# abdel-habib/mmg-clip

Hardware: AMD Instinct MI355X
Metric: image-text pairs/sec (global batch) (higher is better)
Workload: dtype bf16; 1 GPU; C2: train_binary_class_clf, ConvNeXt-tiny 1024x1024x1 + BERT-base S=77, LinearProjection 768->512, CLIPLoss, AdamW, all parameters trained; global_batch=256, per_gpu_batch=256, micro_batch=256, streams=text tower on a side stream, parallelism=dp1, loss_scope=local, text_dropout=HF training-mode dropout live (hidden 0.1, atte…

## Files before the change

### include/mmgclip_hip.h

```cpp
#ifndef MMGCLIP_HIP_H
#define MMGCLIP_HIP_H

#ifdef __cplusplus
extern "C" {
#endif

typedef void* mmg_stream_t;

int mmg_abi_version(void);
const char* mmg_last_error(void);
const char* mmg_target_arch(void);
int mmg_device_cu_count(void);
int mmg_set_kernel_notes(int on);
const char* mmg_last_kernel(void);
const char* mmg_gemm_plan(int op, int M, int N, int K, int cus);


int mmg_l2norm_fwd(const float* x, float* y, float* norm, int rows, int D, mmg_stream_t stream);
int mmg_l2norm_bwd(const float* y, const float* norm, const float* dy, float* dx, int rows, int D,
                   mmg_stream_t stream);

int mmg_clip_rows_fwd(const float* X, const float* Y, const float* scale, int n_loc, int N, int D, int diag_off,
                      float* lse, float* pos, float* logits, int ldl, mmg_stream_t stream);

// ... 38 lines not shown

int mmg_gelu_fwd_bf16(const void* x, void* y, long long n, mmg_stream_t stream);
int mmg_act_grad_bf16(const void* dy, const void* pre, void* out, long long n, int kind, mmg_stream_t stream);
int mmg_cast_f32_bf16(const float* x, void* y, long long n, mmg_stream_t stream);
int mmg_cast_bf16_f32(const void* x, float* y, long long n, mmg_stream_t stream);
int mmg_transpose_cast_bf16(const float* src, int R, int C, const float* rowscale, void* dst, int ldd,
                            mmg_stream_t stream);

int mmg_avgpool_fwd(const void* x, float* y, int n, int HW, int C, mmg_stream_t stream);
int mmg_avgpool_bwd(const float* dy, void* dx, int n, int HW, int C, mmg_stream_t stream);

int mmg_view_pool_fwd(const float* feat, const int* offsets, float* out, int* argmax, int S, int C, int mode, mmg_stream_t stream);
int mmg_view_pool_bwd(const float* dout, const int* offsets, const int* argmax, float* dfeat, int S, int V, int C, int mode,
                      mmg_stream_t stream);

int mmg_patchify(const float* img, void* out, int n, int Cin, int H, int W, int P, int Kp, int scale16,
                 mmg_stream_t stream);
int mmg_patchify_aug(const void* img, int src_kind, void* out, int n, int Cin, int H, int W, int P, int Kp, int scale16,
                     const int* geom, const float* tone, mmg_stream_t stream);

int mmg_adamw_step(float* p, const float* g, float* m, float* v, void* p_bf16, long long n, float lr, float beta1,
                   float beta2, float eps, float weight_decay, int step, float grad_scale, mmg_stream_t stream);


int mmg_grad_sumsq_partials(long long n);
int mmg_grad_sumsq(const float* g, long long n, double* partials, int n_partials, mmg_stream_t stream);
int mmg_grad_clip_finalize(const double* partials, int n, float max_norm, float* out, int* skipped, mmg_stream_t stream);
int mmg_adamw_step_guarded(float* p, const float* g, float* m, float* v, void* p_bf16, long long n, float lr, float beta1,
                           float beta2, float eps, float weight_decay, int step, const float* clip, const int* skipped,
                           mmg_stream_t stream);
int mmg_adamw_step_groups(float* p, const float* g, float* m, float* v, long long n, const unsigned char* chunk_group, int n_groups,
                          const float* group_lr, const float* group_wd, float beta1, float beta2, float eps, int step,
                          const float* clip, const int* skipped, mmg_stream_t stream);

int mmg_layerscale_finalize(const float* W2, const float* b2, const float* gamma, const float* dW2raw,
                            const float* db2raw, float* dW2, float* db2, float* dgamma, int C, int K,
                            mmg_stream_t stream);
int mmg_grad_relayout(const float* src, float* dst, int mode, int R, int CI, int KH, int KW, int ld_src,
                      mmg_stream_t stream);

int mmg_image_swap(void* x, const int* pairs, const int* pairs_host, int k, int n, long long rows, int C, mmg_stream_t stream);
int mmg_image_copy(const void* src, void* dst, int first, int count, int n, long long rows, int C, mmg_stream_t stream);
int mmg_scaled_add_f32(float* dst, const float* src, float alpha, long long n, mmg_stream_t stream);

int mmg_dropout_fwd(const float* x, float* y, void* keep, long long n, float p, long long seed, mmg_stream_t stream);
int mmg_dropout_bwd(const float* dy, const void* keep, float* dx, long long n, float p, mmg_stream_t stream);


int mmg_dwconv7_nhwc(const void* x, const float* w, const float* bias, const void* add, void* y, int n, int H, int W,
                     int C, int flip, mmg_stream_t stream);
int mmg_dwconv7_nhwc_mfma(const void* x, const float* w, const float* bias, const void* add, void* y, int n, int H, int W,
                          int C, int flip, mmg_stream_t stream);
int mmg_dwconv7_wgrad(const void* x, const void* dy, float* dw, float* dbias, int n, int H, int W, int C,
                      mmg_stream_t stream);


long long mmg_cnblock_packed_elems(int C, int backward);
int mmg_cnblock_pack_weights(const float* w1, const float* w2, const float* gamma, void* packed, int C, int backward,
                             mmg_stream_t stream);
int mmg_cnblock_mlp_fwd(const void* xd, const float* ln_w, const float* ln_b, float eps, const void* packed,
                        const float* b1, const float* b2, const float* gamma, const void* residual, void* y, void* hpre,
                        void* xln, void* gact, float* mean, float* rstd, int hpre_kind, long long M, int C, mmg_stream_t stream);

int mmg_cnblock_mlp_bwd_supported(int C);
int mmg_cnblock_mlp_bwd(const void* dy, const void* xd, const float* ln_w, const float* ln_b, float eps,
                        const void* packed_bwd, const float* b1, const void* hpre, void* dh, void* g, void* xln,
                        void* dxln, float* mean, float* rstd, float* ln_dw, float* ln_db, long long M, int C,
                        mmg_stream_t stream);

int mmg_cnblock_bwdw_supported(int C);
long long mmg_cnblock_bwdw_packed_elems(int C);
int mmg_cnblock_bwdw_pack(const float* w1, const float* w2, const float* ln_w, const float* ln_b, const float* layer_scale,
                          const float* b1, void* packed, float* b1f, int C, mmg_stream_t stream);
int mmg_cnblock_bwdw(const void* dy, const void* xd, const float* ln_w, const float* ln_b, float eps, const void* packed,
                     const float* b1f, void* dd, float* dW1, float* db1, float* dW2raw, float* db2raw, float* ln_dw,
                     float* ln_db, long long M, int C, mmg_stream_t stream);

int mmg_stem_supported(int C, int kp);
int mmg_stem_fwd(const void* p0, const void* w, const float* bias, const float* ln_w, const float* ln_b, float eps, void* x,
                 float* mean, float* rstd, long long M, int C, int kp, mmg_stream_t stream);
int mmg_stem_bwd(const void* dx, const void* p0, const void* w, const float* bias, const float* ln_w, const float* mean,
                 const float* rstd, float* dW, float* db, float* ln_dw, float* ln_db, long long M, int C, int kp,
                 mmg_stream_t stream);


int mmg_greedy_threshold_labels(const float* sim, int ld, int n, float threshold, long long* labels, int* counts, int* k_out,
                                mmg_stream_t stream);

int mmg_cluster_mean_cols_fwd(const float* logits, int ld, int n, int N, const long long* labels, const int* counts, int k,
                              float* out, int ldo, mmg_stream_t stream);
int mmg_cluster_mean_cols_bwd(const float* dout, int ldo, int n, int N, const long long* labels, const int* counts,
                              float* dlogits, int ld, mmg_stream_t stream);

int mmg_clip_labelled_rows_fwd(const float* X, const float* Y, const float* scale, const long long* row_label, int n_loc, int M,
                               int D, float* lse, float* pos, mmg_stream_t stream);
int mmg_clip_labelled_rows_bwd_row(const float* X, const float* Y, const float* scale, const float* lse_row,
                                   const long long* row_label, const float* gout, float coef, int n_loc, int M, int D,
                                   int accumulate, float* dX, float* dscale, mmg_stream_t stream);
int mmg_clip_labelled_rows_bwd_col(const float* X, const float* Y, const float* scale, const float* lse_col,
                                   const long long* col_label, const long long* row_key, int key_off, const int* counts,
                                   int n_counts, const float* gout, float coef, int n_loc, int M, int D, int accumulate,
                                   float* dX, mmg_stream_t stream);
int mmg_cluster_centroids(const float* T, const long long* labels, int N, int D, int k, float* out, mmg_stream_t stream);


int mmg_gemm_nt_fp8(const void* A, int lda, const void* B, int ldb, void* C, int ldc, int M, int N, int K,
                    const float* bias, const float* colscale, const void* residual, int ldr, void* aux_out, int ldao,
                    int epi, int out_kind, float alpha, const float* alpha_dev, mmg_stream_t stream);


int mmg_quantize_e5m2_bf16(const void* src, long long n, float* amax, void* dst, float* scales, mmg_stream_t stream);
int mmg_quantize_e5m2_bf16_delayed(const void* src, long long n, const float* amax_prev, float* amax_next, void* dst, float* scales,
                                   mmg_stream_t stream);
int mmg_quantize_e5m2_colsum_bf16(const void* src, int M, int C, const float* amax_prev, float* amax_next, void* dst, float* scales,
                                  float* colsum, mmg_stream_t stream);
int mmg_gemm_nt_fp8_bwd(const void* A, int lda, int a_e5m2, const void* B, int ldb, void* C, int ldc, int M, int N, int K,
                        const void* aux_in, int ldai, int epi, int out_kind, float alpha, const float* alpha_dev,
                        const float* alpha_dev2, mmg_stream_t stream);
int mmg_gemm_tn_fp8(const void* A, int lda, int a_e5m2, const void* B, int ldb, float* C, int ldc, int M, int N1, int N2,
                    float alpha, const float* alpha_dev, float* colsum_a, mmg_stream_t stream);

int mmg_absmax_f32(const float* src, long long n, float* amax, mmg_stream_t stream);
int mmg_quantize_e4m3_f32(const float* src, long long n, const float* amax, void* dst, float* scales, mmg_stream_t stream);

int mmg_layernorm_fwd_fp8(const void* x, int ldx, const float* gamma, const float* beta, float eps, void* y8, int ldy,
                          float* mean, float* rstd, int M, int C, mmg_stream_t stream);


int mmg_im2col_nhwc(const void* x, void* col, int n, int H, int W, int C, int KH, int KW, int stride, int pad, int Kp,
                    mmg_stream_t stream);
int mmg_col2im_nhwc(const void* dcol, void* dx, int n, int H, int W, int C, int KH, int KW, int stride, int pad, int Kp,
                    mmg_stream_t stream);
int mmg_maxpool3x3s2_nhwc(const void* x, void* y, int n, int H, int W, int C, mmg_stream_t stream);
int mmg_bn_stats_f64(const void* x, int M, int C, double* sum, double* sumsq, mmg_stream_t stream);
int mmg_bn_finalize_f64(const double* sum, const double* sumsq, int M, int C, const float* gamma, const float* beta, float eps,
                        float momentum, float* running_mean, float* running_var, int train, float* mean, float* rstd,
                        float* scale, float* shift, mmg_stream_t stream);
int mmg_bn_apply(const void* x, const float* scale, const float* shift, const void* residual, void* y, int M, int C, int relu,
                 mmg_stream_t stream);
int mmg_bn_bwd_reduce(const void* dy, const void* x, const void* out, const float* mean, const float* rstd, int M, int C,
                      float* sum_g, float* sum_gx, mmg_stream_t stream);
int mmg_bn_bwd_apply(const void* dy, const void* x, const void* out, const float* mean, const float* rstd, const float* gamma,
                     const float* sum_g, const float* sum_gx, int M, int C, void* dx, void* dres, float* dgamma, float* dbeta,
                     mmg_stream_t stream);


int mmg_attention_fwd(const void* qkv, int ld, const long long* mask, void* ctx, int ldc, float* lse, int B, int S,
                      int heads, int Hd, float scale, mmg_stream_t stream);
int mmg_attention_bwd(const void* qkv, int ld, const long long* mask, const void* ctx, int ldc, const float* lse,
                      const void* dctx, int lddc, void* dqkv, int lddq, int B, int S, int heads, int Hd, float scale,
                      mmg_stream_t stream);

int mmg_attention_long_fwd(const void* qkv, int ld, const long long* mask, void* ctx, int ldc, float* lse, int B, int S,
                           int heads, int Hd, float scale, mmg_stream_t stream);
int mmg_attention_long_bwd(const void* qkv, int ld, const long long* mask, const void* ctx, int ldc, const float* lse,
                           const void* dctx, int lddc, void* dqkv, int lddq, float* delta_ws, int B, int S, int heads,
                           int Hd, float scale, mmg_stream_t stream);

int mmg_attention_varlen_fwd(const void* qkv, int ld, const int* cu_seqlens, void* ctx, int ldc, float* lse, int B, int S_max,
                             int heads, int Hd, float scale, mmg_stream_t stream);
int mmg_attention_varlen_bwd(const void* qkv, int ld, const int* cu_seqlens, const void* ctx, int ldc, const float* lse,
                             const void* dctx, int lddc, void* dqkv, int lddq, int B, int S_max, int heads, int Hd,
                             float scale, mmg_stream_t stream);

int mmg_attention_dropout_fwd(const void* qkv, int ld, const long long* mask, const int* cu_seqlens, void* ctx, int ldc,
                              float* lse, int B, int S, int heads, int Hd, float scale, float p, unsigned long long seed,
// ... 35 lines not shown
```

### mmg-clip_amd/mmgclip/kernels.py

```python
import ctypes
import os

import torch

from . import _hip
from ._hip import call, ptr, stream
from .profile import PROFILE

BF16 = torch.bfloat16


def layernorm_fwd(x, gamma, beta, eps, patch_hw=None, want_stats=True):
    M, C = x.shape
    if patch_hw is None:
        y = torch.empty(M, C, device=x.device, dtype=BF16)
        patch, H, W = 0, 0, 0
    else:
        H, W = patch_hw
        y = torch.empty((M // (H * W)) * (H // 2) * (W // 2), 4 * C, device=x.device, dtype=BF16)
        patch = 1
    mean = torch.empty(M, device=x.device, dtype=torch.float32) if want_stats else None
    rstd = torch.empty(M, device=x.device, dtype=torch.float32) if want_stats else None
    PROFILE.timed("layernorm_fwd_kernel", 8.0 * M * C, 4 * M * C,
                  lambda: call("mmg_layernorm_fwd", ptr(x), x.stride(0), ptr(gamma), ptr(beta), float(eps), ptr(y), y.stride(0), ptr(mean),
# ... 152 lines not shown


def view_pool_fwd(feat, offsets, S, mode, out=None, argmax=None):
    V, C = feat.shape
    assert feat.dtype == torch.float32 and feat.is_contiguous() and offsets.dtype == torch.int32 and offsets.numel() == S + 1
    _hip.require_gpu(feat, offsets)
    y = out if out is not None else torch.empty(S, C, device=feat.device, dtype=torch.float32)
    if mode == 1 and argmax is None:
        argmax = torch.empty(S, C, device=feat.device, dtype=torch.int32)
    call("mmg_view_pool_fwd", ptr(feat), ptr(offsets), ptr(y), ptr(argmax) if mode == 1 else None, S, C, mode, stream())
    return y, (argmax if mode == 1 else None)


def view_pool_bwd(dout, offsets, argmax, V, mode, out=None):
    S, C = dout.shape
    assert dout.dtype == torch.float32 and dout.is_contiguous() and offsets.dtype == torch.int32 and offsets.numel() == S + 1
    _hip.require_gpu(dout, offsets)
    dx = out if out is not None else torch.empty(V, C, device=dout.device, dtype=torch.float32)
    call("mmg_view_pool_bwd", ptr(dout), ptr(offsets), ptr(argmax), ptr(dx), S, V, C, mode, stream())
    return dx


PIXEL_KINDS = {torch.float32: 0, torch.uint16: 1, torch.uint8: 2}


def stack_images(images):
    if images[0].dtype == torch.uint16:
        return torch.stack([t.view(torch.int16) for t in images]).view(torch.uint16)
    return torch.stack(list(images))


def patchify(img, P, Kp, scale16, geom=None, tone=None):
    n, Cin, H, W = img.shape
    if img.dtype not in PIXEL_KINDS:
        raise TypeError(f"pixels must be float32 in [0, 1], uint16 or uint8, got {img.dtype}")
    assert img.is_contiguous(), "pixels must be contiguous [n, Cin, H, W]"
    _hip.require_gpu(img, geom, tone)
    out = torch.empty(n * (H // P) * (W // P), Kp, device=img.device, dtype=BF16)
    if img.dtype == torch.float32 and geom is None and tone is None:
        call("mmg_patchify", ptr(img), ptr(out), n, Cin, H, W, P, Kp, 1 if scale16 else 0, stream())
        return out
    assert geom is None or (geom.dtype == torch.int32 and geom.is_contiguous() and tuple(geom.shape) == (n, 4)), "geom: int32 [n, 4]"
    assert tone is None or (tone.dtype == torch.float32 and tone.is_contiguous() and tuple(tone.shape) == (n, 2)), "tone: fp32 [n, 2]"
    call("mmg_patchify_aug", ptr(img), PIXEL_KINDS[img.dtype], ptr(out), n, Cin, H, W, P, Kp, 1 if scale16 else 0, ptr(geom), ptr(tone),
         stream())
    return out


def stem_supported(C, kp):
    return bool(_hip.load().mmg_stem_supported(int(C), int(kp)))


def stem_fused_enabled():
    return os.environ.get("MMG_STEM_FUSED", "1") != "0"


def stem_fwd(p0, w, bias, ln_w, ln_b, eps, want_stats=True):
    M, kp = p0.shape
    C = w.shape[0]
    assert p0.dtype == BF16 and w.dtype == BF16 and p0.is_contiguous() and w.is_contiguous() and w.shape[1] == kp
    _hip.require_gpu(p0, w, bias, ln_w, ln_b)
    x = torch.empty(M, C, device=p0.device, dtype=BF16)
    mean = torch.empty(M, device=p0.device, dtype=torch.float32) if want_stats else None
    rstd = torch.empty(M, device=p0.device, dtype=torch.float32) if want_stats else None
    PROFILE.timed("stem_fwd_kernel", 2.0 * M * C * kp, 2 * M * (kp + C) + (8 * M if want_stats else 0) + 2 * C * kp,
                  lambda: call("mmg_stem_fwd", ptr(p0), ptr(w), ptr(bias), ptr(ln_w), ptr(ln_b), float(eps), ptr(x), ptr(mean), ptr(rstd),
                               M, C, kp, stream()), f"M={M} C={C} kp={kp}" + (" +stats" if want_stats else ""))
    return x, mean, rstd


def stem_bwd(dx, p0, w, bias, ln_w, mean, rstd, dW, db, ln_dw, ln_db):
    M, kp = p0.shape
    C = w.shape[0]
    assert dx.dtype == BF16 and p0.dtype == BF16 and dx.is_contiguous() and p0.is_contiguous() and tuple(dx.shape) == (M, C)
    assert mean.dtype == rstd.dtype == torch.float32 and mean.numel() == rstd.numel() == M
    for t, n in ((dW, C * kp), (db, C), (ln_dw, C), (ln_db, C)):
        assert t.dtype == torch.float32 and t.is_contiguous() and t.numel() == n
    _hip.require_gpu(dx, p0, w, bias, ln_w, mean, rstd, dW, db, ln_dw, ln_db)
    PROFILE.timed("stem_bwd_kernel", 2.0 * M * C * kp, 2 * M * (kp + C) + 8 * M + 6 * C * kp,
                  lambda: call("mmg_stem_bwd", ptr(dx), ptr(p0), ptr(w), ptr(bias), ptr(ln_w), ptr(mean), ptr(rstd), ptr(dW), ptr(db),
                               ptr(ln_dw), ptr(ln_db), M, C, kp, stream()), f"M={M} C={C} kp={kp}")


def adamw_step(p, g, m, v, p16, lr, beta1, beta2, eps, wd, step, grad_scale=1.0):
    call("mmg_adamw_step", ptr(p), ptr(g), ptr(m), ptr(v), ptr(p16), p.numel(), float(lr), float(beta1), float(beta2),
         float(eps), float(wd), int(step), float(grad_scale), stream())


def grad_sumsq_partials(n):
    return int(_hip.load().mmg_grad_sumsq_partials(int(n)))


def grad_sumsq(g, partials, offset=0, count=None):
    assert g.dtype == torch.float32 and g.is_contiguous() and partials.dtype == torch.float64 and partials.is_contiguous()
    _hip.require_gpu(g, partials)
    count = grad_sumsq_partials(g.numel()) if count is None else int(count)
    assert 0 <= offset and offset + count <= partials.numel()
    call("mmg_grad_sumsq", ptr(g), g.numel(), ptr(partials[offset:]) if count else ptr(partials), count, stream())


def grad_clip_finalize(partials, n, max_norm, out, skipped=None):
    assert partials.dtype == torch.float64 and out.dtype == torch.float32 and out.numel() >= 3 and n <= partials.numel()
    assert skipped is None or (skipped.dtype == torch.int32 and skipped.numel() >= 1)
    _hip.require_gpu(partials, out, skipped)
    call("mmg_grad_clip_finalize", ptr(partials), int(n), 0.0 if max_norm is None else float(max_norm), ptr(out), ptr(skipped), stream())


def adamw_step_guarded(p, g, m, v, p16, lr, beta1, beta2, eps, wd, step, clip, skipped=None):
    assert clip.dtype == torch.float32 and clip.numel() >= 3 and (skipped is None or skipped.dtype == torch.int32)
    call("mmg_adamw_step_guarded", ptr(p), ptr(g), ptr(m), ptr(v), ptr(p16), p.numel(), float(lr), float(beta1), float(beta2),
         float(eps), float(wd), int(step), ptr(clip), ptr(skipped), stream())


ADAMW_MAX_GROUPS = 128


def adamw_step_groups(p, g, m, v, chunk_group, group_lr, group_wd, beta1, beta2, eps, step, clip=None, skipped=None):
    n_groups = len(group_lr)
    assert len(group_wd) == n_groups and chunk_group.dtype == torch.uint8 and chunk_group.is_contiguous()
    assert chunk_group.numel() * 64 == p.numel() == g.numel() == m.numel() == v.numel()
    assert clip is None or (clip.dtype == torch.float32 and clip.numel() >= 3)
    assert skipped is None or skipped.dtype == torch.int32
    _hip.require_gpu(p, g, m, v, chunk_group, clip, skipped)
    lrs = (ctypes.c_float * max(n_groups, 1))(*[float(x) for x in group_lr])
    wds = (ctypes.c_float * max(n_groups, 1))(*[float(x) for x in group_wd])
    call("mmg_adamw_step_groups", ptr(p), ptr(g), ptr(m), ptr(v), p.numel(), ptr(chunk_group), n_groups, lrs, wds, float(beta1),
         float(beta2), float(eps), int(step), ptr(clip), ptr(skipped), stream())


def dwconv_mfma_pays(n, H, W, C, flip):
    return H * W >= 96 * 96 and C <= 256


def dwconv7(x, w49, bias, n, H, W, C, add=None, flip=False, out=None):
    y = out if out is not None else torch.empty(n * H * W, C, device=x.device, dtype=BF16)
    px = n * H * W * C
    mode = os.environ.get("MMG_DWCONV_MFMA", "auto")
    if mode == "1" or (mode == "auto" and dwconv_mfma_pays(n, H, W, C, flip)):
        PROFILE.timed("dwconv7_mfma_kernel", 98.0 * px, (6 if add is not None else 4) * px,
                      lambda: call("mmg_dwconv7_nhwc_mfma", ptr(x), ptr(w49), ptr(bias), ptr(add), ptr(y), n, H, W, C, 1 if flip else 0, stream()),
                      f"n={n} {H}x{W} C={C}" + (" +add" if add is not None else ""))
        return y
    fam = "dwconv7_rows2_kernel" if os.environ.get("MMG_DWCONV_ROWS2", "1") != "0" else "dwconv7_kernel"
    PROFILE.timed(fam, 98.0 * px, (6 if add is not None else 4) * px,
                  lambda: call("mmg_dwconv7_nhwc", ptr(x), ptr(w49), ptr(bias), ptr(add), ptr(y), n, H, W, C, 1 if flip else 0, stream()),
                  f"n={n} {H}x{W} C={C}" + (" +add" if add is not None else ""))
    return y


def dwconv7_wgrad(x, dy, dw49, dbias, n, H, W, C):
    px = n * H * W * C
    fam = "dwconv7_wgrad_rows2_kernel" if os.environ.get("MMG_DWCONV_ROWS2", "1") != "0" else "dwconv7_wgrad_kernel"
    PROFILE.timed(fam, 98.0 * px, 4 * px,
                  lambda: call("mmg_dwconv7_wgrad", ptr(x), ptr(dy), ptr(dw49), ptr(dbias), n, H, W, C, stream()), f"n={n} {H}x{W} C={C}")


def cnblock_supported(C):
    return C in (96, 128, 192, 256, 384, 512)


def cnblock_pack(w1, w2, gamma=None, backward=False):
    C = w1.shape[1]
    backward = int(backward)
    n = _hip.load().mmg_cnblock_packed_elems(C, backward)
    if n <= 0:
        raise ValueError(f"fused CNBlock MLP: C={C} is not supported")
# ... 225 lines not shown
```

### mmg-clip_amd/mmgclip/networks/convnext.py

```python
import ctypes
import os

import torch
import torch.nn as nn

from .. import _hip
from .. import kernels as K
from .. import linalg as L
from .._hip import call, ptr, stream
from ..params import backward_finished, last_backward
from . import convnext_sd as SD
from .convnext_plan import BlockSaved, Knobs, decide_saves, fused_forward, plan_block, saving_form
from .tower import Tower, as_pixels, augment_tables, backward_parts, conv_weight_rows, fold_conv_grad, forward_parts

CONFIGS = {
    "tiny": dict(depths=(3, 3, 9, 3), dims=(96, 192, 384, 768)),
    "small": dict(depths=(3, 3, 27, 3), dims=(96, 192, 384, 768)),
    "base": dict(depths=(3, 3, 27, 3), dims=(128, 256, 512, 1024)),
}
LN_EPS = 1e-6


def _fused_save_maxc():
    return int(os.environ.get("MMG_MLP_FUSED_SAVE_MAXC", "384"))


class LayerNorm2d(nn.LayerNorm):
    """Parameter container with torchvision's name; the arithmetic runs in mmg_layernorm_fwd."""


class CNBlock(nn.Module):
    def __init__(self, dim, layer_scale=1e-6):
        super().__init__()
        self.block = nn.Sequential(
            nn.Conv2d(dim, dim, kernel_size=7, padding=3, groups=dim, bias=True),
            nn.Identity(),
            nn.LayerNorm(dim, eps=LN_EPS),
            nn.Linear(dim, 4 * dim, bias=True),
            nn.GELU(),
            nn.Linear(4 * dim, dim, bias=True),
            nn.Identity(),
        )
        self.layer_scale = nn.Parameter(torch.ones(dim, 1, 1) * layer_scale)


def build_features(variant="tiny", in_chans=1):
    cfg = CONFIGS[variant]
    dims, depths = cfg["dims"], cfg["depths"]
    layers = [nn.Sequential(nn.Conv2d(in_chans, dims[0], kernel_size=4, stride=4, bias=True), LayerNorm2d(dims[0], eps=LN_EPS))]
    for i, (d, n) in enumerate(zip(dims, depths)):
        layers.append(nn.Sequential(*[CNBlock(d) for _ in range(n)]))
        if i < 3:
            layers.append(nn.Sequential(LayerNorm2d(d, eps=LN_EPS), nn.Conv2d(d, dims[i + 1], kernel_size=2, stride=2)))
    feats = nn.Sequential(*layers)
    for m in feats.modules():
        if isinstance(m, (nn.Conv2d, nn.Linear)):
            nn.init.trunc_normal_(m.weight, std=0.02)
            if m.bias is not None:
                nn.init.zeros_(m.bias)
    return feats


class _TorchvisionLayout(nn.Module):

    def __init__(self, variant, in_chans):
        super().__init__()
        self.features = build_features(variant, in_chans)
        self.avgpool = nn.AdaptiveAvgPool2d(1)


class ConvNextTower(Tower):

    def __init__(self, variant="tiny", in_chans=1, scale16=True, micro_batch=64, fused_mlp=None, checkpoint=False, fp8=False,
                 fp8_min_channels=None, stochastic_depth_prob=0.0, augment=None):
        super().__init__()
        self.set_augment(augment)
        self.stochastic_depth_prob = SD.check_rate(stochastic_depth_prob)
        self.next_drop_seed = None
        self._drop_seeds = SD.DropSeeds()
        self.variant, self.in_chans, self.scale16, self.micro_batch = variant, in_chans, scale16, micro_batch
        self.fused_mlp = (os.environ.get("MMG_FUSED_MLP", "1") != "0") if fused_mlp is None else bool(fused_mlp)
        self.fused_bwd_saved_h = os.environ.get("MMG_FUSED_MLP_BWD_SAVED_H", "0") == "1"
        self.bwdw = os.environ.get("MMG_BWDW", "1") != "0"
        self.save_ln_mode = os.environ.get("MMG_SAVE_LN", "auto")
        self.save_ln = self.save_ln_mode == "1"
        self.save_gelu_mode = os.environ.get("MMG_SAVE_GELU", "auto")
        self.save_gelu = self.save_gelu_mode == "1"
        self.save_dgelu = os.environ.get("MMG_SAVE_DGELU", "1") != "0"
        self.checkpoint = checkpoint
        self.fp8 = bool(fp8)
        self.fp8_bwd_mode = os.environ.get("MMG_FP8_BWD", "auto")
        self.fp8_bwd = self.fp8_bwd_mode != "0"
        self.fp8_bwd_now = False
        self.fp8_delayed = os.environ.get("MMG_FP8_DELAYED", "1") != "0"
        self._e5m2_state = {}
        self.fp8_min_channels = int(os.environ.get("MMG_FP8_MIN_C", "256" if self.fp8_bwd else "512")) if fp8_min_channels is None else int(fp8_min_channels)
        self.dims, self.depths = CONFIGS[variant]["dims"], CONFIGS[variant]["depths"]
        self.model = _TorchvisionLayout(variant, in_chans)
        self.model_output_dimension = self.dims[-1]
        self.kp = (16 * in_chans + 31) // 32 * 32
        self.plan = None

    def _bound(self):
        self._pname = {id(m): "features." + n for n, m in self.model.features.named_modules()}

    def _g(self, mod, leaf):
        return self._arena.g(self._pname[id(mod)] + "." + leaf)
# ... 114 lines not shown
            s0 = L.gemm_nt(p0, wc["stem.w"], bias=f[0][0].bias.data)
            x, mean, rstd = K.layernorm_fwd(s0, f[0][1].weight.data, f[0][1].bias.data, LN_EPS, want_stats=save)
        if save:
            saved["stem"] = (p0, s0, mean, rstd)
        for si, p in enumerate(plan):
            mlp = self._fwd_fused if fused_forward(p, save) else self._fwd_gemm
            for bi, blk in enumerate(f[1 + 2 * si]):
                key = f"{si}.{bi}"
                step = steps[b] if steps is not None else None
                b += 1
                if step is None or step.n_k == n:
                    d = K.dwconv7(x, wc[key + ".w49"], blk.block[0].bias.data, n, h, w_, p.C)
                    x, rec = mlp(x, d, blk, key, p, dec)
                elif step.n_k == 0:
                    rec = None
                else:
                    K.image_swap_(x, n, *(table or (None, None)), len(step.pairs), step.offset)
                    n_k, Mk = step.n_k, step.n_k * h * w_
                    xk, out = x[:Mk], torch.empty_like(x)
                    d = K.dwconv7(xk, wc[key + ".w49"], blk.block[0].bias.data, n_k, h, w_, p.C)
                    _, rec = mlp(xk, d, blk, key, p, dec, out=out[:Mk])
                    K.image_copy(x, out, n, n_k, n - n_k)
                    x = out
                if save:
                    saved[key] = rec
            if si < 3:
                lnm = f[2 + 2 * si][0]
                ld, mean, rstd = K.layernorm_fwd(x, lnm.weight.data, lnm.bias.data, LN_EPS, patch_hw=(h, w_), want_stats=save)
                xn = L.gemm_nt(ld, wc[f"ds{si}.w"], bias=f[2 + 2 * si][1].bias.data)
                if save:
                    saved[f"ds{si}"] = (x, mean, rstd, ld)
                x = xn
                h, w_ = h // 2, w_ // 2
                saved["maps"].append((h, w_))
        feat = K.avgpool_fwd(x, n, h * w_, self.dims[-1])
        saved["shape"] = (n, H, W)
        return feat, saved

    def _ln_bwd(self, dln, d, mean, rstd, blk):
        return K.layernorm_bwd(dln, d, mean, rstd, blk.block[2].weight.data, self._g(blk.block[2], "weight"), self._g(blk.block[2], "bias"))

    def _bwd_bwdw(self, dx, rec, blk, key, tmp):
        packed, b1f = self._wc[key + ".bwdw"]
        return K.cnblock_bwdw(dx, rec.d, blk.block[2].weight.data, blk.block[2].bias.data, LN_EPS, packed, b1f,
                              self._g(blk.block[3], "weight"), self._g(blk.block[3], "bias"), tmp[key + ".dw2raw"], tmp[key + ".db2raw"],
                              self._g(blk.block[2], "weight"), self._g(blk.block[2], "bias"))

    def _bwd_fused(self, dx, rec, blk, key, tmp):
        fuse_ln = rec.d.shape[1] <= 128
        dh, g, ln, dln, mean, rstd = K.cnblock_mlp_bwd(
            dx, rec.d, blk.block[2].weight.data, blk.block[2].bias.data, LN_EPS, self._wc[key + ".mlpb"], blk.block[3].bias.data, rec.aux,
            ln_grads=(self._g(blk.block[2], "weight"), self._g(blk.block[2], "bias")) if fuse_ln else None)
        L.gemm_tn_acc(dx, g, tmp[key + ".dw2raw"], colsum=tmp[key + ".db2raw"])
        del g
        L.gemm_tn_acc(dh, ln, self._g(blk.block[3], "weight"), colsum=self._g(blk.block[3], "bias"))
        del ln, dh
        return dln if fuse_ln else self._ln_bwd(dln, rec.d, mean, rstd, blk)

    def _bwd_fp8(self, dx, rec, blk, key, tmp):
        wc = self._wc
        dy8, sdy = K.quantize_e5m2(dx, self._e5m2_state.setdefault(key, {}) if self.fp8_delayed else None, colsum=tmp[key + ".db2raw"])
        dh8 = L.gemm_nt_fp8_bwd(dy8, wc[key + ".w2gt8"], aux_in=rec.aux, epi=L.EPI_MUL_AUX, out_kind=L.OUT_E5M2,
                                alpha_dev=wc[key + ".s2gt"][1:])
        L.gemm_tn_fp8_acc(dy8, rec.g, tmp[key + ".dw2raw"], alpha_dev=sdy[1:])
        L.gemm_tn_fp8_acc(dh8, rec.ln, self._g(blk.block[3], "weight"), alpha_dev=sdy[1:], colsum=self._g(blk.block[3], "bias"))
        dln = L.gemm_nt_fp8_bwd(dh8, wc[key + ".w1t8"], alpha_dev=wc[key + ".s1t"][1:], alpha_dev2=sdy[1:])
        del dh8, dy8
        return self._ln_bwd(dln, rec.d, rec.mean, rec.rstd, blk)

    def _bwd_gemm(self, dx, rec, blk, key, tmp):
        wc = self._wc
        if rec.g is not None:
            g = rec.g
            dh = L.gemm_nt(dx, wc[key + ".w2gt"], epi=L.EPI_MUL_AUX if rec.aux_kind == "dgelu" else L.EPI_DGELU_ONLY, aux_in=rec.aux)
        else:
            g = torch.empty_like(rec.aux)
            dh = L.gemm_nt(dx, wc[key + ".w2gt"], epi=L.EPI_DGELU, aux_in=rec.aux, aux_out=g)
        L.gemm_tn_acc(dx, g, tmp[key + ".dw2raw"], colsum=tmp[key + ".db2raw"])
        del g
        ln = rec.ln if rec.ln is not None else \
            K.layernorm_fwd(rec.d, blk.block[2].weight.data, blk.block[2].bias.data, LN_EPS, want_stats=False)[0]
        L.gemm_tn_acc(dh, ln, self._g(blk.block[3], "weight"), colsum=self._g(blk.block[3], "bias"))
        del ln
        dln = L.gemm_nt(dh, wc[key + ".w1t"])
        del dh
        return self._ln_bwd(dln, rec.d, rec.mean, rec.rstd, blk)

    def _backward_mb(self, dfeat, saved, tmp, final=False, announce=False):
        f, wc, A = self.model.features, self._wc, self._arena
        n, H, W = saved["shape"]
        maps = saved["maps"]
        steps, table = saved.get("sd", (None, None))
        b = sum(self.depths)
        h, w_ = maps[3]
        dx = K.avgpool_bwd(dfeat, n, h * w_, self.dims[-1])
        for si in range(3, -1, -1):
            C = self.dims[si]
            if si < 3:
                x, mean, rstd, ld = saved[f"ds{si}"]
                conv, lnm = f[2 + 2 * si][1], f[2 + 2 * si][0]
                L.gemm_tn_acc(dx, ld, tmp[f"ds{si}.dw"], colsum=self._g(conv, "bias"))
                dld = L.gemm_nt(dx, wc[f"ds{si}.wt"])
                h, w_ = maps[si]
                dx = K.layernorm_bwd(dld, x, mean, rstd, lnm.weight.data, self._g(lnm, "weight"), self._g(lnm, "bias"),
                                     patch_hw=(h, w_))
                del dld
            for bi in range(self.depths[si] - 1, -1, -1):
                blk = f[1 + 2 * si][bi]
                key = f"{si}.{bi}"
                rec = saved[key]
                b -= 1
                step = steps[b] if steps is not None else None
                if step is None or step.n_k == n:
                    dd = getattr(self, "_bwd_" + rec.bwd)(dx, rec, blk, key, tmp)
                    K.dwconv7_wgrad(rec.x, dd, tmp[key + ".dw49"], self._g(blk.block[0], "bias"), n, h, w_, C)
                    dx = K.dwconv7(dd, wc[key + ".w49"], None, n, h, w_, C, add=dx, flip=True)
                    del dd
                elif step.n_k:
                    n_k, Mk = step.n_k, step.n_k * h * w_
                    dxk, dxn = dx[:Mk], torch.empty_like(dx)
                    dd = getattr(self, "_bwd_" + rec.bwd)(dxk, rec, blk, key, tmp)
                    K.dwconv7_wgrad(rec.x, dd, tmp[key + ".dw49"], self._g(blk.block[0], "bias"), n_k, h, w_, C)
                    K.dwconv7(dd, wc[key + ".w49"], None, n_k, h, w_, C, add=dxk, flip=True, out=dxn[:Mk])
                    del dd, dxk
                    K.image_copy(dx, dxn, n, n_k, n - n_k)
                    dx = K.image_swap_(dxn, n, *(table or (None, None)), len(step.pairs), step.offset)
            if final:
                self._finalize_stage(tmp, si)
                if announce:
                    A.mark_ready((f"features.{1 + 2 * si}.",) + ((f"features.{2 + 2 * si}.",) if si < 3 else ()))
        p0, s0, mean, rstd = saved["stem"]
        if s0 is None:
            K.stem_bwd(dx, p0, wc["stem.w"], f[0][0].bias.data, f[0][1].weight.data, mean, rstd, tmp["stem.dw"], self._g(f[0][0], "bias"),
                       self._g(f[0][1], "weight"), self._g(f[0][1], "bias"))
        else:
            ds0 = K.layernorm_bwd(dx, s0, mean, rstd, f[0][1].weight.data, self._g(f[0][1], "weight"), self._g(f[0][1], "bias"))
            L.gemm_tn_acc(ds0, p0, tmp["stem.dw"], colsum=self._g(f[0][0], "bias"))
        if final:
            fold_conv_grad(tmp["stem.dw"], self._g(f[0][0], "weight"), self.dims[0], self.in_chans, 4, 4)

    def _alloc_tmp(self, device):
        z = lambda *s: torch.zeros(*s, device=device, dtype=torch.float32)
        tmp = {"stem.dw": z(self.dims[0], self.kp)}
        for si in range(4):
            C = self.dims[si]
            for bi in range(self.depths[si]):
                key = f"{si}.{bi}"
                tmp[key + ".dw2raw"], tmp[key + ".db2raw"], tmp[key + ".dw49"] = z(C, 4 * C), z(C), z(49, C)
            if si < 3:
                tmp[f"ds{si}.dw"] = z(self.dims[si + 1], 4 * C)
        return tmp

    def _finalize_stage(self, tmp, si):
        f = self.model.features
        C = self.dims[si]
        scales = self._wc["sd.scales"]
        for bi, blk in enumerate(f[1 + 2 * si]):
            key = f"{si}.{bi}"
            s = scales[sum(self.depths[:si]) + bi] if scales is not None else 1.0
            dgamma = self._g(blk, "layer_scale") if s == 1.0 else torch.zeros(C, device=tmp[key + ".dw2raw"].device, dtype=torch.float32)
            call("mmg_layerscale_finalize", ptr(blk.block[5].weight.data), ptr(blk.block[5].bias.data),
                 ptr(self._wc[key + ".gamma"]), ptr(tmp[key + ".dw2raw"]), ptr(tmp[key + ".db2raw"]),
                 ptr(self._g(blk.block[5], "weight")), ptr(self._g(blk.block[5], "bias")),
                 ptr(dgamma), C, 4 * C, stream())
            if s != 1.0:
                K.scaled_add_(self._g(blk, "layer_scale"), dgamma, s)
            call("mmg_grad_relayout", ptr(tmp[key + ".dw49"]), ptr(self._g(blk.block[0], "weight")), 1, C, 1, 7, 7, C,
                 stream())
        if si < 3:
            fold_conv_grad(tmp[f"ds{si}.dw"], self._g(f[2 + 2 * si][1], "weight"), self.dims[si + 1], C, 2, 2)

    def feature_map_shape(self, H, W):
        h, w = H // 4, W // 4
        for _ in range(3):
            h, w = h // 2, w // 2
        return h, w

    def forward(self, images, sample_ids=None):
        plan = None
        if isinstance(images, (list, tuple)):
            if not images or any(not torch.is_tensor(t) or t.dim() != 3 for t in images):
                raise ValueError("a list of images must hold [Cin, H, W] tensors")
            for t in images:
                _hip.require_gpu(t)
                if t.shape[-2] < 32 or t.shape[-1] < 32:
                    raise ValueError(f"ConvNeXt needs at least 32x32 pixels, got {tuple(t.shape)}")
            plan = group_by_size([tuple(t.shape[-2:]) for t in images], self.micro_batch)
            device = images[0].device
        else:
# ... 102 lines not shown
```

Before: 888.0 image-text pairs/sec.

## Fuse NT GEMM with LayerNorm backward in ConvNeXt block and downsample backward

Adds a HIP kernel that runs the dgrad GEMM (dh·W1ᵀ or the downsample dx·Wᵀ) and applies the LayerNorm backward on the output tile still held in LDS. It also accumulates dgamma and dbeta in the same kernel, optionally with the patchified (2x2 downsample) pixel mapping. This removes the round trip of the bf16 intermediate through HBM and a separate layernorm_bwd launch. The GEMM output is rounded to bf16 in LDS before the LN math. The GEMM tile shape is fixed at 128x384 on a persistent grid, which may run slower than the general GEMM. The path is on by default and falls back to the old one for unsupported shapes.

```diff
diff --git a/include/mmgclip_hip.h b/include/mmgclip_hip.h
--- a/include/mmgclip_hip.h
+++ b/include/mmgclip_hip.h
@@ -144,6 +144,11 @@
 int mmg_stem_bwd(const void* dx, const void* p0, const void* w, const float* bias, const float* ln_w, const float* mean,
                  const float* rstd, float* dW, float* db, float* ln_dw, float* ln_db, long long M, int C, int kp,
                  mmg_stream_t stream);
+
+int mmg_gemm_nt_lnbwd_supported(int N, int K, int C, int patch, int H, int W);
+int mmg_gemm_nt_lnbwd(const void* A, int lda, const void* B, int ldb, int M, int N, int K, const void* x, int ldx,
+                      const float* mean, const float* rstd, const float* gamma, void* dx, int lddx, float* dgamma, float* dbeta,
+                      int C, int patch, int H, int W, mmg_stream_t stream);
 
 
 int mmg_greedy_threshold_labels(const float* sim, int ld, int n, float threshold, long long* labels, int* counts, int* k_out,
diff --git a/mmg-clip_amd/csrc/gemm_lnbwd.hip b/mmg-clip_amd/csrc/gemm_lnbwd.hip
--- /dev/null
+++ b/mmg-clip_amd/csrc/gemm_lnbwd.hip
@@ -0,0 +1,313 @@
+#include "common.h"
+
+#define LNB_BM 128
+#define LNB_BN 384
+#define LNB_BK 64
+#define LNB_THREADS 512
+#define LNB_STAGE ((LNB_BM + LNB_BN) * LNB_BK * 2)
+#define LNB_PITCH (LNB_BN * 2 + 16)
+#define LNB_RED (2 * LNB_STAGE)
+#define LNB_GAM (LNB_RED + 2 * LNB_BN * 4)
+#define LNB_LDS (LNB_GAM + LNB_BN * 4)
+static_assert(LNB_BM * LNB_PITCH <= 2 * LNB_STAGE, "the tile image aliases the two stages");
+static_assert(LNB_LDS <= 160 * 1024, "LDS of a CU");
+
+struct GemmLnBwd {
+    const bf16_t* A; const bf16_t* B;
+    int M, N, K, lda, ldb;
+    const bf16_t* x; int ldx;
+    const float* mean; const float* rstd; const float* gamma;
+    bf16_t* dx; int lddx;
+    float* dgamma; float* dbeta;
+    int H, W;
+    int tiles_n, tiles;
+    int nt;
+};
+
+__device__ __forceinline__ void lnb_glds16(const void* gsrc, void* lds_wave_base) {
+    __builtin_amdgcn_global_load_lds((const __attribute__((address_space(1))) void*)gsrc,
+                                     (__attribute__((address_space(3))) void*)lds_wave_base, 16, 0, 0);
+}
+
+template <int G>
+__device__ __forceinline__ float lnb_group_sum(float v) {
+    if (G >= 2) v += __int_as_float(__builtin_amdgcn_mov_dpp(__float_as_int(v), 0xB1, 0xf, 0xf, true));
+    if (G >= 4) v += __int_as_float(__builtin_amdgcn_mov_dpp(__float_as_int(v), 0x4E, 0xf, 0xf, true));
+    if (G >= 8) v += __int_as_float(__builtin_amdgcn_mov_dpp(__float_as_int(v), 0x141, 0xf, 0xf, true));
+    if (G >= 16) v += __int_as_float(__builtin_amdgcn_mov_dpp(__float_as_int(v), 0x140, 0xf, 0xf, true));
+    return v;
+}
+
+__device__ __forceinline__ void lnb_unpack8(const uint4 v, float* f) {
+    f[0] = bf2f_lo(v.x); f[1] = bf2f_hi(v.x); f[2] = bf2f_lo(v.y); f[3] = bf2f_hi(v.y);
+    f[4] = bf2f_lo(v.z); f[5] = bf2f_hi(v.z); f[6] = bf2f_lo(v.w); f[7] = bf2f_hi(v.w);
+}
+
+template <int C, int PATCH>
+__global__ __launch_bounds__(LNB_THREADS, 1) void gemm_nt_lnbwd_kernel(const GemmLnBwd g) {
+    static_assert(C == 96 || C == 192 || C == 384, "a 384-column tile holds whole pixels");
+    static_assert(PATCH == 1 || C == LNB_BN, "plain rows: N = C = one column tile");
+    constexpr int BM = LNB_BM, BN = LNB_BN, BK = LNB_BK, THREADS = LNB_THREADS;
+    constexpr int MI = 4, NI = 6;
+    constexpr int A_BYTES = BM * BK * 2, STAGE = LNB_STAGE;
+    constexpr int CPR = BK / 8;
+    constexpr int A_IT = BM * CPR / THREADS, B_IT = BN * CPR / THREADS;
+    constexpr int G = C / 24, CH = 3;
+    constexpr int SEG = BN / C;
+    constexpr int PASSES = BM / 32;
+    constexpr int PRE = 1, POST = PASSES - PRE;
+    extern __shared__ __attribute__((aligned(16))) char smem[];
+
+    const int tid = threadIdx.x, wave = tid >> 6, lane = tid & 63;
+    const int wm = wave >> 2, wn = wave & 3;
+    const int li = lane & 15, lg = lane >> 4;
+    const int gi = lane / G, gl = lane % G;
+    const int prow = wave * 4 + gi / SEG, seg = gi % SEG;
+
+    float* red = reinterpret_cast<float*>(smem + LNB_RED);
+    float* sgam = reinterpret_cast<float*>(smem + LNB_GAM);
+    for (int i = tid; i < 2 * C; i += THREADS) red[i] = 0.f;
+    for (int i = tid; i < C; i += THREADS) sgam[i] = g.gamma[i];
+
+    const unsigned b_off = (unsigned)((tid / CPR) * g.ldb + ((tid % CPR) ^ ((tid / CPR) & 7)) * 8) * 2u;
+    const size_t b_step = (size_t)(THREADS / CPR) * g.ldb * 2;
+    char* lds_wave = smem + (tid & ~63) * 16;
+    int a_frag[BK / 32], b_frag[BK / 32];
+#pragma unroll
+    for (int ks = 0; ks < BK / 32; ++ks) {
+        const int ra = wm * 64 + li, rb = wn * 96 + li;
+        a_frag[ks] = ra * (BK * 2) + (((4 * ks + lg) ^ (ra & 7)) << 4);
+        b_frag[ks] = A_BYTES + rb * (BK * 2) + (((4 * ks + lg) ^ (rb & 7)) << 4);
+    }
+    const int nk = g.K / BK;
+    const float inv_c = 1.0f / (float)C;
+
+    float dg[CH][8], db[CH][8];
+#pragma unroll
+    for (int k = 0; k < CH; ++k)
+#pragma unroll
+        for (int e = 0; e < 8; ++e) { dg[k][e] = 0.f; db[k][e] = 0.f; }
+
+    const int t_begin = (int)((long long)blockIdx.x * g.tiles / gridDim.x), t_end = (int)((long long)(blockIdx.x + 1) * g.tiles / gridDim.x);
+    for (int t = t_begin; t < t_end; ++t) {
+        const int tm = t / g.tiles_n, tn = t - tm * g.tiles_n;
+        const int m0 = tm * BM, n0 = tn * BN;
+        const int s = n0 / C + seg;
+
+        unsigned a_off[A_IT];
+#pragma unroll
+        for (int it = 0; it < A_IT; ++it) {
+            const int p = it * THREADS + tid, r = p / CPR, sl = p % CPR;
+            const int gr = min(m0 + r, g.M - 1) - m0;
+            a_off[it] = (unsigned)(gr * g.lda + (sl ^ (r & 7)) * 8) * 2u;
+        }
+        const char* a_base = reinterpret_cast<const char*>(g.A + (size_t)m0 * g.lda);
+        const char* b_base = reinterpret_cast<const char*>(g.B + (size_t)n0 * g.ldb);
+        auto stage = [&](int buf, int kt) {
+            const char* ab = a_base + (size_t)kt * (BK * 2);
+            const char* bb = b_base + (size_t)kt * (BK * 2);
+            char* la = lds_wave + buf * STAGE;
+#pragma unroll
+            for (int it = 0; it < A_IT; ++it) lnb_glds16(ab + a_off[it], la + it * THREADS * 16);
+#pragma unroll
+            for (int it = 0; it < B_IT; ++it) lnb_glds16(bb + it * b_step + b_off, la + A_BYTES + it * THREADS * 16);
+        };
+        stage(0, 0);
+
+        int pix[PASSES];
+#pragma unroll
+        for (int p = 0; p < PASSES; ++p) {
+            const int r = min(m0 + p * 32 + prow, g.M - 1);
+            if constexpr (PATCH) {
+                const int w2 = g.W >> 1, h2 = g.H >> 1;
+                const int pw = r % w2, ph = (r / w2) % h2, n = r / (w2 * h2);
+                pix[p] = (n * g.H + 2 * ph + (s >> 1)) * g.W + 2 * pw + (s & 1);
+            } else {
+                pix[p] = r;
+            }
+        }
+        uint4 xa[PRE][CH], xb[POST][CH];
+        float mua[PRE], rsa[PRE], mub[POST], rsb[POST];
+#pragma unroll
+        for (int p = 0; p < PRE; ++p) {
+#pragma unroll
+            for (int k = 0; k < CH; ++k) xa[p][k] = *reinterpret_cast<const uint4*>(g.x + (size_t)pix[p] * g.ldx + (gl + k * G) * 8);
+            mua[p] = g.mean[pix[p]];
+            rsa[p] = g.rstd[pix[p]];
+        }
+
+        f32x4 acc[MI][NI];
+#pragma unroll
+        for (int i = 0; i < MI; ++i)
+#pragma unroll
+            for (int j = 0; j < NI; ++j) acc[i][j] = f32x4{0.f, 0.f, 0.f, 0.f};
+
+        for (int kt0 = 0; kt0 < nk; kt0 += 2) {
+#pragma unroll
+            for (int sb = 0; sb < 2; ++sb) {
+                const int kt = kt0 + sb;
+                if (kt < nk) {
+                    asm volatile("s_waitcnt vmcnt(0)" ::: "memory");
+                    __syncthreads();
+                    if (kt + 1 < nk) stage(sb ^ 1, kt + 1);
+                    const char* buf = smem + sb * STAGE;
+#pragma unroll
+                    for (int ks = 0; ks < BK / 32; ++ks) {
+                        bf16x8 af[MI], bfr[NI];
+#pragma unroll
+                        for (int i = 0; i < MI; ++i) af[i] = *reinterpret_cast<const bf16x8*>(buf + a_frag[ks] + i * 16 * BK * 2);
+#pragma unroll
+                        for (int j = 0; j < NI; ++j) bfr[j] = *reinterpret_cast<const bf16x8*>(buf + b_frag[ks] + j * 16 * BK * 2);
+#pragma unroll
+                        for (int i = 0; i < MI; ++i)
+#pragma unroll
+                            for (int j = 0; j < NI; ++j)
+                                acc[i][j] = __builtin_amdgcn_mfma_f32_16x16x32_bf16(bfr[j], af[i], acc[i][j], 0, 0, 0);
+                    }
+                }
+            }
+        }
+
+        asm volatile("s_waitcnt lgkmcnt(0)\n\ts_barrier" ::: "memory");
+#pragma unroll
+        for (int i = 0; i < MI; ++i)
+#pragma unroll
+            for (int j = 0; j < NI; ++j)
+                *reinterpret_cast<uint2*>(smem + (wm * 64 + i * 16 + li) * LNB_PITCH + (wn * 96 + j * 16 + 4 * lg) * 2) =
+                    make_uint2(pack2bf(acc[i][j][0], acc[i][j][1]), pack2bf(acc[i][j][2], acc[i][j][3]));
+        __builtin_amdgcn_sched_barrier(0);
+#pragma unroll
+        for (int p = 0; p < POST; ++p) {
+#pragma unroll
+            for (int k = 0; k < CH; ++k) xb[p][k] = *reinterpret_cast<const uint4*>(g.x + (size_t)pix[PRE + p] * g.ldx + (gl + k * G) * 8);
+            mub[p] = g.mean[pix[PRE + p]];
+            rsb[p] = g.rstd[pix[PRE + p]];
+        }
+        asm volatile("s_waitcnt lgkmcnt(0)\n\ts_barrier" ::: "memory");
+
+        float gam[CH][8];
+#pragma unroll
+        for (int k = 0; k < CH; ++k) {
+            const int c = gl + k * G;
+            const float4 g0 = *reinterpret_cast<const float4*>(sgam + c * 8), g1 = *reinterpret_cast<const float4*>(sgam + c * 8 + 4);
+            gam[k][0] = g0.x; gam[k][1] = g0.y; gam[k][2] = g0.z; gam[k][3] = g0.w; gam[k][4] = g1.x; gam[k][5] = g1.y; gam[k][6] = g1.z; gam[k][7] = g1.w;
+        }
+        auto row_pass = [&](int p, const uint4* xr, float mu, float rs) {
+            const int rl = p * 32 + prow;
+            const bool live = m0 + rl < g.M;
+            uint4 dr[CH];
+#pragma unroll
+            for (int k = 0; k < CH; ++k) {
+                dr[k] = *reinterpret_cast<const uint4*>(smem + rl * LNB_PITCH + (seg * C + (gl + k * G) * 8) * 2);
+                if (!live) dr[k] = make_uint4(0u, 0u, 0u, 0u);
+            }
+            float s1 = 0.f, s2 = 0.f;
+#pragma unroll
+            for (int k = 0; k < CH; ++k) {
+                float xv[8], dyv[8];
+                lnb_unpack8(xr[k], xv);
+                lnb_unpack8(dr[k], dyv);
+#pragma unroll
+                for (int e = 0; e < 8; ++e) {
+                    const float xh = (xv[e] - mu) * rs, gg = dyv[e] * gam[k][e];
+                    s1 += gg;
+                    s2 += gg * xh;
+                    dg[k][e] += dyv[e] * xh;
+                    db[k][e] += dyv[e];
+                }
+            }
+#pragma unroll
+            for (int k = 0; k < CH; ++k)
+#pragma unroll
+                for (int e = 0; e < 8; ++e) asm volatile("" : "+v"(dg[k][e]), "+v"(db[k][e]));
+            s1 = lnb_group_sum<G>(s1) * inv_c;
+            s2 = lnb_group_sum<G>(s2) * inv_c;
+#pragma unroll
+            for (int k = 0; k < CH; ++k) {
+                float xv[8], dyv[8], o[8];
+                lnb_unpack8(xr[k], xv);
+                lnb_unpack8(dr[k], dyv);
+#pragma unroll
+                for (int e = 0; e < 8; ++e) o[e] = rs * (dyv[e] * gam[k][e] - s1 - (xv[e] - mu) * rs * s2);
+                if (live)
+                    store16_stream(g.dx + (size_t)pix[p] * g.lddx + (gl + k * G) * 8,
+                                   make_uint4(pack2bf(o[0], o[1]), pack2bf(o[2], o[3]), pack2bf(o[4], o[5]), pack2bf(o[6], o[7])), g.nt != 0);
+            }
+        };
+#pragma unroll
+        for (int p = 0; p < PRE; ++p) row_pass(p, xa[p], mua[p], rsa[p]);
+#pragma unroll
+        for (int p = 0; p < POST; ++p) row_pass(PRE + p, xb[p], mub[p], rsb[p]);
+        asm volatile("s_waitcnt lgkmcnt(0)\n\ts_barrier" ::: "memory");
+    }
+
+    if (g.dgamma) {
+#pragma unroll
+        for (int k = 0; k < CH; ++k)
+#pragma unroll
+            for (int e = 0; e < 8; ++e) {
+                atomicAdd(&red[(gl + k * G) * 8 + e], dg[k][e]);
+                atomicAdd(&red[C + (gl + k * G) * 8 + e], db[k][e]);
+            }
+        __syncthreads();
+        for (int i = tid; i < C; i += THREADS) {
+            atomicAdd(g.dgamma + i, red[i]);
+            atomicAdd(g.dbeta + i, red[C + i]);
+        }
+    }
+}
+
+static const char* lnb_shape_error(int N, int K, int C, int patch, int H, int W) {
+    if (!(C == 96 || C == 192 || C == 384)) return "C must be 96, 192 or 384";
+    if (!(patch == 0 || patch == 1)) return "patch must be 0 or 1";
+    if (N <= 0 || N % LNB_BN != 0) return "N must be a positive multiple of 384";
+    if (K < LNB_BK || K % LNB_BK != 0) return "K must be a positive multiple of 64";
+    if (patch == 0 && N != C) return "plain rows need N == C";
+    if (patch == 1 && N != 4 * C) return "patchified rows need N == 4 C";
+    if (patch == 1 && (H < 2 || W < 2 || (H & 1) || (W & 1))) return "patchified rows need even H and W (odd maps: the two-launch path)";
+    return nullptr;
+}
+
+MMG_API int mmg_gemm_nt_lnbwd_supported(int N, int K, int C, int patch, int H, int W) {
+    return lnb_shape_error(N, K, C, patch, H, W) == nullptr ? 1 : 0;
+}
+
+template <int C, int PATCH>
+static void lnb_launch(const GemmLnBwd& g, hipStream_t stream) {
+    const int cus = mmg_cu_count_cached();
+    mmg_allow_lds(gemm_nt_lnbwd_kernel<C, PATCH>, LNB_LDS);
+    MMG_NOTE_KERNEL("gemm_nt_lnbwd_kernel<%d, %d>", C, PATCH);
+    hipLaunchKernelGGL((gemm_nt_lnbwd_kernel<C, PATCH>), dim3(g.tiles < cus ? g.tiles : cus), dim3(LNB_THREADS), LNB_LDS, stream, g);
+}
+
+MMG_API int mmg_gemm_nt_lnbwd(const void* A, int lda, const void* B, int ldb, int M, int N, int K, const void* x, int ldx,
+                              const float* mean, const float* rstd, const float* gamma, void* dx, int lddx, float* dgamma, float* dbeta,
+                              int C, int patch, int H, int W, hipStream_t stream) {
+    const char* why = lnb_shape_error(N, K, C, patch, H, W);
+    MMG_CHECK_ARG(why == nullptr, "mmg_gemm_nt_lnbwd: N=%d K=%d C=%d patch=%d H=%d W=%d is not supported: %s", N, K, C, patch, H, W, why ? why : "");
+    MMG_CHECK_ARG(M >= 1, "mmg_gemm_nt_lnbwd: M=%d must be positive", M);
+    MMG_CHECK_ARG(patch == 0 || M % ((H / 2) * (W / 2)) == 0,
+                  "mmg_gemm_nt_lnbwd: M=%d is not supported: not a multiple of the (H/2)(W/2) = %d patch rows of an image", M, (H / 2) * (W / 2));
+    MMG_CHECK_ARG((long long)M * (patch ? 4 : 1) <= 0x7fffffffLL, "mmg_gemm_nt_lnbwd: M=%d has too many pixels", M);
+    MMG_CHECK_ARG(lda >= K && ldb >= K && ldx >= C && lddx >= C, "mmg_gemm_nt_lnbwd: a leading dimension is shorter than its row (lda=%d ldb=%d K=%d ldx=%d lddx=%d C=%d)",
+                  lda, ldb, K, ldx, lddx, C);
+    MMG_CHECK_ARG(lda % 8 == 0 && ldb % 8 == 0 && ldx % 8 == 0 && lddx % 8 == 0, "mmg_gemm_nt_lnbwd: leading dimensions must be multiples of 8 (16-byte rows)");
+    MMG_CHECK_ARG((long long)LNB_BM * lda * 2 <= 0x7fffffffLL && (long long)LNB_BN * ldb * 2 <= 0x7fffffffLL, "mmg_gemm_nt_lnbwd: lda=%d / ldb=%d too large", lda, ldb);
+    MMG_CHECK_ARG(A && B && x && mean && rstd && gamma && dx, "mmg_gemm_nt_lnbwd: null pointer");
+    MMG_CHECK_ARG((dgamma == nullptr) == (dbeta == nullptr), "mmg_gemm_nt_lnbwd: dgamma and dbeta are accumulated together (both or neither)");
+    MMG_CHECK_ARG((((uintptr_t)A | (uintptr_t)B | (uintptr_t)x | (uintptr_t)dx) & 15) == 0, "mmg_gemm_nt_lnbwd: A, B, x and dx must be 16-byte aligned");
+    const long long tiles = (long long)cdiv(M, LNB_BM) * (N / LNB_BN);
+    MMG_CHECK_ARG(tiles <= 0x7fffffffLL, "mmg_gemm_nt_lnbwd: too many tiles");
+    GemmLnBwd g;
+    g.A = (const bf16_t*)A; g.B = (const bf16_t*)B; g.M = M; g.N = N; g.K = K; g.lda = lda; g.ldb = ldb;
+    g.x = (const bf16_t*)x; g.ldx = ldx; g.mean = mean; g.rstd = rstd; g.gamma = gamma; g.dx = (bf16_t*)dx; g.lddx = lddx;
+    g.dgamma = dgamma; g.dbeta = dbeta; g.H = H; g.W = W;
+    g.tiles_n = N / LNB_BN; g.tiles = (int)tiles;
+    g.nt = (size_t)M * N * 2 >= ((size_t)256 << 20) ? 1 : 0;
+    if (patch == 0) lnb_launch<384, 0>(g, stream);
+    else if (C == 96) lnb_launch<96, 1>(g, stream);
+    else if (C == 192) lnb_launch<192, 1>(g, stream);
+    else lnb_launch<384, 1>(g, stream);
+    MMG_LAUNCH_CHECK("mmg_gemm_nt_lnbwd");
+    return 0;
+}
diff --git a/mmg-clip_amd/mmgclip/kernels.py b/mmg-clip_amd/mmgclip/kernels.py
--- a/mmg-clip_amd/mmgclip/kernels.py
+++ b/mmg-clip_amd/mmgclip/kernels.py
@@ -258,6 +258,32 @@
                                ptr(ln_dw), ptr(ln_db), M, C, kp, stream()), f"M={M} C={C} kp={kp}")
 
 
+def gemm_nt_lnbwd_supported(N, K, C, patch_hw=None):
+    patch, H, W = (0, 0, 0) if patch_hw is None else (1, int(patch_hw[0]), int(patch_hw[1]))
+    return bool(_hip.load().mmg_gemm_nt_lnbwd_supported(int(N), int(K), int(C), patch, H, W))
+
+
+def lnbwd_fused_enabled():
+    return os.environ.get("MMG_LNBWD_FUSED", "1") != "0"
+
+
+def gemm_nt_lnbwd(a, b, x, mean, rstd, gamma, dgamma=None, dbeta=None, patch_hw=None, out=None):
+    M, Kd = a.shape
+    N = b.shape[0]
+    P, C = x.shape
+    patch, H, W = (0, 0, 0) if patch_hw is None else (1, int(patch_hw[0]), int(patch_hw[1]))
+    assert a.dtype == BF16 and b.dtype == BF16 and x.dtype == BF16 and b.shape[1] == Kd
+    assert P == (4 * M if patch else M) and mean.numel() == rstd.numel() == P and mean.dtype == rstd.dtype == torch.float32
+    assert a.stride(1) == 1 and b.stride(1) == 1 and x.stride(1) == 1
+    _hip.require_gpu(a, b, x, mean, rstd, gamma, dgamma, dbeta, out)
+    dx = out if out is not None else torch.empty(P, C, device=x.device, dtype=BF16)
+    PROFILE.timed("gemm_nt_lnbwd_kernel", 2.0 * M * N * Kd, 2 * M * Kd + 2 * N * Kd + 4 * M * N + 8 * P + 12 * C,
+                  lambda: call("mmg_gemm_nt_lnbwd", ptr(a), a.stride(0), ptr(b), b.stride(0), M, N, Kd, ptr(x), x.stride(0), ptr(mean),
+                               ptr(rstd), ptr(gamma), ptr(dx), dx.stride(0), ptr(dgamma), ptr(dbeta), C, patch, H, W, stream()),
+                  f"M={M} N={N} K={Kd} C={C}" + (" patchified" if patch else ""))
+    return dx
+
+
 def adamw_step(p, g, m, v, p16, lr, beta1, beta2, eps, wd, step, grad_scale=1.0):
     call("mmg_adamw_step", ptr(p), ptr(g), ptr(m), ptr(v), ptr(p16), p.numel(), float(lr), float(beta1), float(beta2),
          float(eps), float(wd), int(step), float(grad_scale), stream())
diff --git a/mmg-clip_amd/mmgclip/networks/convnext.py b/mmg-clip_amd/mmgclip/networks/convnext.py
--- a/mmg-clip_amd/mmgclip/networks/convnext.py
+++ b/mmg-clip_amd/mmgclip/networks/convnext.py
@@ -23,6 +23,10 @@
 
 def _fused_save_maxc():
     return int(os.environ.get("MMG_MLP_FUSED_SAVE_MAXC", "384"))
+
+
+def lnbwd_fused(M, N, Kd, C, patch_hw=None):
+    return K.lnbwd_fused_enabled() and K.gemm_nt_lnbwd_supported(N, Kd, C, patch_hw)
 
 
 class LayerNorm2d(nn.LayerNorm):
@@ -303,7 +307,12 @@
             K.layernorm_fwd(rec.d, blk.block[2].weight.data, blk.block[2].bias.data, LN_EPS, want_stats=False)[0]
         L.gemm_tn_acc(dh, ln, self._g(blk.block[3], "weight"), colsum=self._g(blk.block[3], "bias"))
         del ln
-        dln = L.gemm_nt(dh, wc[key + ".w1t"])
+        w1t, lnm = wc[key + ".w1t"], blk.block[2]
+        if lnbwd_fused(dh.shape[0], w1t.shape[0], w1t.shape[1], rec.d.shape[1]):
+            dd = K.gemm_nt_lnbwd(dh, w1t, rec.d, rec.mean, rec.rstd, lnm.weight.data, self._g(lnm, "weight"), self._g(lnm, "bias"))
+            del dh
+            return dd
+        dln = L.gemm_nt(dh, w1t)
         del dh
         return self._ln_bwd(dln, rec.d, rec.mean, rec.rstd, blk)
 
@@ -321,11 +330,16 @@
                 x, mean, rstd, ld = saved[f"ds{si}"]
                 conv, lnm = f[2 + 2 * si][1], f[2 + 2 * si][0]
                 L.gemm_tn_acc(dx, ld, tmp[f"ds{si}.dw"], colsum=self._g(conv, "bias"))
-                dld = L.gemm_nt(dx, wc[f"ds{si}.wt"])
+                wt = wc[f"ds{si}.wt"]
                 h, w_ = maps[si]
-                dx = K.layernorm_bwd(dld, x, mean, rstd, lnm.weight.data, self._g(lnm, "weight"), self._g(lnm, "bias"),
-                                     patch_hw=(h, w_))
-                del dld
+                if lnbwd_fused(dx.shape[0], wt.shape[0], wt.shape[1], C, (h, w_)):
+                    dx = K.gemm_nt_lnbwd(dx, wt, x, mean, rstd, lnm.weight.data, self._g(lnm, "weight"), self._g(lnm, "bias"),
+                                         patch_hw=(h, w_))
+                else:
+                    dld = L.gemm_nt(dx, wt)
+                    dx = K.layernorm_bwd(dld, x, mean, rstd, lnm.weight.data, self._g(lnm, "weight"), self._g(lnm, "bias"),
+                                         patch_hw=(h, w_))
+                    del dld
             for bi in range(self.depths[si] - 1, -1, -1):
                 blk = f[1 + 2 * si][bi]
                 key = f"{si}.{bi}"
```

Result: faster. 905.2 image-text pairs/sec, median of 6 (+1.9%).
